# shellrow/nex

Measured on AMD Instinct MI355X. Metric: Mpkt/s + GiB/s device-resident parse+cksum, 64B & IMIX, 1/2/4/8 MI355X, higher is better.
Workload: dtype u8

## Files before the change

### nex_amd/csrc/frame_core.hpp

```cpp
#pragma once

#include <hip/hip_runtime.h>
#include <stdint.h>

#include "../../include/nexg.h"

#define NEXG_HD __host__ __device__ __forceinline__

namespace nexg {

NEXG_HD uint32_t ip_next_protocol_value(uint32_t n) {
    return (n <= 142u || n == 253u || n == 254u) ? n : 255u;
}

NEXG_HD uint32_t fold_complement(uint64_t t) {
    t = (t & 0xFFFFFFFFull) + (t >> 32);
    t = (t & 0xFFFFFFFFull) + (t >> 32);
    uint32_t s = (uint32_t)t;
    s = (s & 0xFFFFu) + (s >> 16);
    s = (s & 0xFFFFu) + (s >> 16);
    return (~s) & 0xFFFFu;
}

#define NEXG_NO_DEFER                                             \
// ... 68 lines not shown

#if defined(__HIP_DEVICE_COMPILE__)
#define NEXG_GLOBAL(T, p) reinterpret_cast<const __attribute__((address_space(1))) T*>(reinterpret_cast<uintptr_t>(p))
#else
#define NEXG_GLOBAL(T, p) reinterpret_cast<const T*>(p)
#endif

template <bool NT = false>
NEXG_HD uint4 load16(const void* p) {
    u32x4 v = NT ? __builtin_nontemporal_load(NEXG_GLOBAL(u32x4, p)) : *NEXG_GLOBAL(u32x4, p);
    return make_uint4(v.x, v.y, v.z, v.w);
}

template <bool NT = false>
NEXG_HD uint4 load16g(uint64_t addr) {
    return load16<NT>(reinterpret_cast<const void*>(addr));
}

NEXG_HD uint64_t global_le_sum(uint64_t A, uint64_t B) {
    uint64_t acc = 0;
    for (uint64_t d = A & ~15ull; d < B; d += 16) {
        const uint4 v = load16(reinterpret_cast<const void*>(d));
        uint32_t s = 0;
        if (d >= A && d + 16 <= B) {
            s = halves(v.x) + halves(v.y) + halves(v.z) + halves(v.w);
        } else {
            if (d + 0 < B) s += halves(v.x & range_mask(d + 0, A, B));
            if (d + 4 < B) s += halves(v.y & range_mask(d + 4, A, B));
            if (d + 8 < B) s += halves(v.z & range_mask(d + 8, A, B));
            if (d + 12 < B) s += halves(v.w & range_mask(d + 12, A, B));
        }
        acc += s;
    }
    return acc;
}

struct WinFrame {
    NEXG_NO_DEFER
    const uint8_t* slot;
    const uint8_t* g;
    uint32_t o;
    uint32_t wlen;

    NEXG_HD uint32_t u8(uint32_t i) const {
        return i < wlen ? (uint32_t)slot[o + i] : (uint32_t)g[i];
    }
    NEXG_HD uint64_t le_sum(uint32_t a, uint32_t b) const {
        uint64_t acc = 0;
        const uint32_t lb = b < wlen ? b : wlen;
        if (a < lb) {
            const uint32_t A = o + a, B = o + lb;
            const uint32_t* w = reinterpret_cast<const uint32_t*>(slot);
            uint32_t s = 0;
            for (uint32_t j = A & ~3u; j < B; j += 4) s += halves(w[j >> 2] & range_mask(j, A, B));
            acc = s;
        }
        const uint32_t ga = a > wlen ? a : wlen;
        if (ga < b) {
            const uint64_t base = reinterpret_cast<uint64_t>(g);
            acc += global_le_sum(base + ga, base + b);
        }
        return acc;
    }
};

struct SpanDeferred {
    uint32_t rng = 0;
    uint32_t t = 0;
    uint32_t meta = 0;
    NEXG_HD uint32_t which() const { return (meta >> 16) & 3u; }
    NEXG_HD uint32_t off() const { return rng & 0xFFFFu; }
    NEXG_HD uint32_t bytes() const { return rng >> 16; }
};

NEXG_HD uint32_t span_tail_end(uint32_t b12, uint32_t b16, uint32_t len, uint32_t opt_flags) {
    if (opt_flags & (NEXG_PARSE_FROM_IP | NEXG_PARSE_VLAN)) return len;
    const uint32_t et = ((b12 & 0xFFu) << 8) | ((b12 >> 8) & 0xFFu);
    const uint32_t e = et == 0x0800u ? 14u + (((b16 & 0xFFu) << 8) | ((b16 >> 8) & 0xFFu))
                     : et == 0x86DDu ? 54u + ((((b16 >> 16) & 0xFFu) << 8) | (b16 >> 24)) : 0u;
    return (e >= 84u && e < len) ? e : len;
}

#ifndef NEXG_SPAN_PROBE
#define NEXG_SPAN_PROBE(k, c)
#endif
#ifndef NEXG_SPAN_SLOT
#define NEXG_SPAN_SLOT 80
#endif
struct SpanFrame {
    static constexpr uint32_t kSlot = NEXG_SPAN_SLOT;
    static_assert(kSlot >= 80 && kSlot % 16 == 0, "the slot holds the 80-B fast-path window");
    static constexpr uint32_t kDefer = 64;
    const uint8_t* slot;
    const uint8_t* g;
    uint32_t tail_end;
    uint32_t parity;
    uint32_t tail;
    mutable SpanDeferred d{};
    mutable bool pend = false;

    NEXG_HD uint32_t u8(uint32_t i) const {
        NEXG_SPAN_PROBE(0, i >= kSlot);
        const uint8_t* p = i < kSlot ? slot + i : g + i;
        return *p;
    }
    NEXG_HD uint64_t le_sum(uint32_t a, uint32_t b) const {
        uint64_t acc = 0;
        const bool to_end = b == tail_end && tail_end > 80u && a <= 80u;
        const uint32_t lb = to_end ? 80u : b < kSlot ? b : kSlot;
        if (a < lb) {
            const uint32_t* w = reinterpret_cast<const uint32_t*>(slot);
            uint32_t s = 0;
            for (uint32_t j = a & ~3u; j < lb; j += 4) s += halves(w[j >> 2] & range_mask(j, a, lb));
            acc = parity ? (uint64_t)s * 256u : (uint64_t)s;
        }
        const uint32_t ga = a > kSlot ? a : kSlot;
        if (!to_end && ga < b) {
            const uint64_t base = reinterpret_cast<uint64_t>(g);
            if (b - ga > kDefer && d.rng == 0) {
                d.rng = ga | (b - ga) << 16;
                pend = true;
            } else {
                NEXG_SPAN_PROBE(1, true);
                acc += global_le_sum(base + ga, base + b);
            }
        }
        if (to_end) acc += tail;
        return acc;
    }
    NEXG_HD void note_mult(uint32_t m) const {
        if (pend) d.meta = (m == 256u ? 1u : 0u) << 18 | 1u << 20;
        pend = false;
    }
    NEXG_HD void note_finish(uint64_t t, uint32_t stored, uint32_t which) const {
        if ((d.meta >> 20) && !d.which()) {
            t = (t & 0xFFFFFFFFull) + (t >> 32);
            d.t = (uint32_t)((t & 0xFFFFFFFFull) + (t >> 32));
            d.meta = (d.meta & (1u << 18)) | which << 16 | (stored & 0xFFFFu);
        }
    }
};

NEXG_HD void span_patch(const SpanDeferred& d, uint64_t range_sum, nexg_record& r) {
    const uint32_t calc = fold_complement((uint64_t)d.t + (((d.meta >> 18) & 1u) ? range_sum * 256u : range_sum));
    const uint32_t stored = d.meta & 0xFFFFu;
    if (d.which() == kCsumIp) {
        r.ip_csum_calc = (uint16_t)calc;
        r.flags = (r.flags & ~NEXG_C_IP_OK) | (calc == stored ? NEXG_C_IP_OK : 0u);
    } else {
        r.l4_csum_calc = (uint16_t)calc;
        r.flags = (r.flags & ~NEXG_C_L4_OK) | (calc == stored ? NEXG_C_L4_OK : 0u);
    }
}


template <class O>
NEXG_HD void parse_udp(const O& o, uint32_t base, uint32_t n,
                                          uint64_t pseudo, nexg_record& r) {
    r.flags |= NEXG_L_TRANSPORT;
    uint32_t ulen = n >= 8 ? o.be16(base + 4) : 0u;
    if (n < 8 || ulen < 8u || n < ulen) {
        set_payload(r, base, n);
        return;
    }
    uint32_t sp = o.be16(base), dp = o.be16(base + 2), cs = o.be16(base + 6);
    r.flags |= NEXG_L_UDP;
    r.l4_off = (uint16_t)base;
    r.src_port = (uint16_t)sp;
    r.dst_port = (uint16_t)dp;
    r.l4_length = (uint16_t)ulen;
    r.l4_csum = (uint16_t)cs;
    uint64_t t = pseudo + 17u + ulen + sp + dp + ulen + o.wsum(base + 8, base + ulen);
    o.finish(t, cs, kCsumL4, r);
    set_payload(r, base + 8, ulen - 8);
}

template <class O>
NEXG_HD void parse_tcp(const O& o, uint32_t base, uint32_t n,
                                          uint64_t pseudo, nexg_record& r) {
    r.flags |= NEXG_L_TRANSPORT;
    bool ok = n >= 20;
    uint32_t off_res = ok ? o.f.u8(base + 12) : 0u;
    uint32_t hl = (off_res >> 4) * 4u;
    ok = ok && hl >= 20u && n >= hl;
    uint32_t stop = hl, nopt = 0;
    if (ok) {
        uint32_t off = 20;
        while (off < hl) {
            uint32_t kind = o.f.u8(base + off);
            off += 1;
            if (kind == 0u) {
                nopt++;
                stop = off;
                break;
            }
            if (kind == 1u) {
                nopt++;
                continue;
            }
            if (off >= hl) { ok = false; break; }
            uint32_t l = o.f.u8(base + off);
            off += 1;
            if (l < 2u) { ok = false; break; }
            if (off + (l - 2u) > hl) { ok = false; break; }
            nopt++;
            off += l - 2u;
        }
    }
    if (!ok) {
        set_payload(r, base, n);
        return;
    }
    uint32_t sp = o.be16(base), dp = o.be16(base + 2);
    uint32_t seq_hi = o.be16(base + 4), seq_lo = o.be16(base + 6);
    uint32_t ack_hi = o.be16(base + 8), ack_lo = o.be16(base + 10);
    uint32_t flags = o.f.u8(base + 13);
    uint32_t win = o.be16(base + 14), cs = o.be16(base + 16), urg = o.be16(base + 18);
    r.flags |= NEXG_L_TCP;
    r.l4_off = (uint16_t)base;
    r.src_port = (uint16_t)sp;
    r.dst_port = (uint16_t)dp;
    r.tcp_seq = (seq_hi << 16) | seq_lo;
    r.tcp_ack = (ack_hi << 16) | ack_lo;
    r.l4_length = (uint16_t)hl;
    r.l4_type = (uint8_t)flags;
    r.l4_code = (uint8_t)off_res;
    r.tcp_window = (uint16_t)win;
    r.tcp_urg = (uint16_t)urg;
    r.l4_nopt = (uint8_t)nopt;
    r.l4_csum = (uint16_t)cs;
    uint32_t hl_ser = 20u + ((stop - 20u + 3u) & ~3u);
    uint32_t len_ser = hl_ser + (n - hl);
    uint64_t t = pseudo + 6u + len_ser + sp + dp + seq_hi + seq_lo + ack_hi + ack_lo +
                 ((((hl_ser >> 2) << 4) | (off_res & 0xFu)) << 8 | flags) + win + urg +
                 o.wsum(base + 20, base + stop) + o.wsum(base + hl, base + n);
    o.finish(t, cs, kCsumL4, r);
    set_payload(r, base + hl, n - hl);
}

template <class O>
NEXG_HD void parse_icmp(const O& o, uint32_t base, uint32_t n,
                                           bool v6, uint64_t pseudo, nexg_record& r) {
    if (n < 8) {
        set_payload(r, base, n);
        return;
    }
    uint32_t tc = o.be16(base), cs = o.be16(base + 2);
    r.flags |= v6 ? NEXG_L_ICMPV6 : NEXG_L_ICMP;
    r.l4_off = (uint16_t)base;
    r.l4_type = (uint8_t)(tc >> 8);
    r.l4_code = (uint8_t)tc;
    r.l4_csum = (uint16_t)cs;
    uint64_t t = (v6 ? pseudo + 58u + n : 0ull) + tc + o.wsum(base + 4, base + n);
    o.finish(t, cs, kCsumL4, r);
    set_payload(r, base + 4, n - 4);
}


template <class O>
NEXG_HD uint32_t parse_ipv4(const O& o, uint32_t l3, uint32_t len,
                                               bool strict, nexg_record& r) {
    const uint32_t n = len - l3;
    r.flags |= NEXG_L_IP;
    uint32_t err = 0, ctx = 0, ea = 0, eb = 0, hl = 0, total = 0;
    uint32_t b0 = n >= 20u ? o.f.u8(l3) : 0u;
    if (n < 20u) { err = NEXG_ERR_BUFFER_TOO_SHORT; ctx = NEXG_CTX_IPV4_PACKET; ea = 20u; eb = n; }
    else if ((b0 >> 4) != 4u) { err = NEXG_ERR_MALFORMED; ctx = NEXG_CTX_IPV4_VERSION; }
    else if ((b0 & 15u) < 5u) { err = NEXG_ERR_INVALID_LENGTH; ctx = NEXG_CTX_IPV4_HEADER_LENGTH; ea = b0 & 15u; }
    else {
        hl = (b0 & 15u) * 4u;
        if (hl > n) { err = NEXG_ERR_TRUNCATED; ctx = NEXG_CTX_IPV4_HEADER; ea = hl; eb = n; }
        else {
            uint32_t declared = o.be16(l3 + 2);
            uint32_t eff = declared ? declared : n;
            if (eff < hl) { err = NEXG_ERR_INVALID_LENGTH; ctx = NEXG_CTX_IPV4_TOTAL_LENGTH; ea = declared; }
            else if (strict && eff > n) { err = NEXG_ERR_TRUNCATED; ctx = NEXG_CTX_IPV4_PACKET; ea = eff; eb = n; }
            else total = eff < n ? eff : n;
        }
    }
    uint32_t stop = hl, nopt = 0;
    if (!err) {
        uint32_t i = 20;
        while (i < hl) {
            uint32_t num = o.f.u8(l3 + i) & 0x1Fu;
            if (num == 0u) { nopt++; stop = i + 1; break; }
            if (num == 1u) { nopt++; i++; continue; }
            if (i + 2u > hl) {
                if (strict) { err = NEXG_ERR_MALFORMED; ctx = NEXG_CTX_IPV4_OPTIONS; }
                stop = i;
                break;
            }
            uint32_t l = o.f.u8(l3 + i + 1);
            if (l < 2u || i + l > hl) {
                if (strict) { err = NEXG_ERR_INVALID_LENGTH; ctx = NEXG_CTX_IPV4_OPTION_LENGTH; ea = l; }
                stop = i;
                break;
            }
            nopt++;
            i += l;
        }
    }
    if (err) {
        if (!strict) return 0u;
        r.l4_type = (uint8_t)ctx;
        r.ip_src = ea;
        r.ip_dst = eb;
// ... 609 lines not shown
```

### nex_amd/csrc/parse_kernels.hpp

```cpp
#pragma once

#include "frame_core.hpp"
#include "nexg_internal.hpp"

namespace nexg {

constexpr uint32_t kTile = 256;

#ifndef NEXG_DESC_MODE
#define NEXG_DESC_MODE 2
#endif
constexpr uint32_t kApron = NEXG_SPAN_SLOT > 96 ? NEXG_SPAN_SLOT : 96;

struct GlobalFrame {
    NEXG_NO_DEFER
    const uint8_t* g;
    NEXG_HD uint32_t u8(uint32_t i) const { return g[i]; }
    NEXG_HD uint64_t le_sum(uint32_t a, uint32_t b) const {
        const uint64_t base = reinterpret_cast<uint64_t>(g);
        return global_le_sum(base + a, base + b);
    }
};

__device__ __forceinline__ uint32_t wave_incl_scan(uint32_t v) {
// ... 365 lines not shown
    }
    if (!__all(fits)) {
        if (have) *handoff_slot<OUT>(a, idx) = (uint32_t)global_le_sum(myA, myA + len - kLaneWin);
        return;
    }
    acc[lane] = 0;
    const uint32_t incl = wave_incl_scan(np);
    pfx[lane] = incl - np;
    const uint32_t total = __shfl(incl, 63, 64);
    if (lane == 63) pfx[64] = total;
    wave_lds_sync();
    const uint32_t grp = lane >> 4, gl = lane & 15u;
    const uint32_t pb = (uint32_t)((uint64_t)total * grp / 4u);
    const uint32_t pe = (uint32_t)((uint64_t)total * (grp + 1u) / 4u);
    const uint8_t* wb = reinterpret_cast<const uint8_t*>(wbase);
    if (pb < pe) {
        uint32_t lo = 0, hi = 64;
        while (hi - lo > 1) {
            const uint32_t mid = (lo + hi) >> 1;
            if (pfx[mid] <= pb) lo = mid; else hi = mid;
        }
        uint32_t fi = lo;
        uint32_t cf = lo, ce = pfx[lo + 1];
        uint32_t ca = tail_a[lo], cb = tail_b[lo];
        uint32_t cpb = (ca & ~(kPiece - 1)) - pfx[lo] * kPiece;
        uint32_t run = 0;
        for (uint32_t p0 = pb; p0 < pe; p0 += PU) {
            uint4 v[PU];
            uint32_t C[PU], AA[PU], BB[PU], F[PU];
#pragma unroll
            for (uint32_t u = 0; u < PU; u++) {
                const uint32_t pp = p0 + u;
                while (pp < pe && pp >= ce) {
                    cf++;
                    ce = pfx[cf + 1];
                    ca = tail_a[cf];
                    cb = tail_b[cf];
                    cpb = (ca & ~(kPiece - 1)) - pfx[cf] * kPiece;
                }
                F[u] = cf;
                AA[u] = ca;
                BB[u] = cb;
                C[u] = cpb + pp * kPiece + 16u * gl;
            }
#pragma unroll
            for (uint32_t u = 0; u < PU; u++) {
                v[u] = make_uint4(0, 0, 0, 0);
                if (p0 + u < pe && C[u] < BB[u] && C[u] + 16u > AA[u]) v[u] = load16<true>(wb + C[u]);
            }
#pragma unroll
            for (uint32_t u = 0; u < PU; u++) {
                if (p0 + u >= pe) break;
                if (F[u] != fi) {
                    uint32_t s = run;
                    s += __shfl_xor(s, 8, 16);
                    s += __shfl_xor(s, 4, 16);
                    s += __shfl_xor(s, 2, 16);
                    s += __shfl_xor(s, 1, 16);
                    if (gl == 0 && s) atomicAdd(&acc[fi], s);
                    run = 0;
                    fi = F[u];
                }
                const uint32_t c = C[u], A = AA[u], B = BB[u];
                if (c < B && c + 16u > A) {
                    if (c >= A && c + 16u <= B) {
                        run += halves(v[u].x) + halves(v[u].y) + halves(v[u].z) + halves(v[u].w);
                    } else {
                        if (c + 0 < B) run += halves(v[u].x & range_mask(c + 0, A, B));
                        if (c + 4 < B) run += halves(v[u].y & range_mask(c + 4, A, B));
                        if (c + 8 < B) run += halves(v[u].z & range_mask(c + 8, A, B));
                        if (c + 12 < B) run += halves(v[u].w & range_mask(c + 12, A, B));
                    }
                }
            }
        }
        uint32_t s = run;
        s += __shfl_xor(s, 8, 16);
        s += __shfl_xor(s, 4, 16);
        s += __shfl_xor(s, 2, 16);
        s += __shfl_xor(s, 1, 16);
        if (gl == 0 && s) atomicAdd(&acc[fi], s);
    }
    wave_lds_sync();
    if (have) *handoff_slot<OUT>(a, idx) = acc[lane];
}

template <int OUT>
__global__ __launch_bounds__(256) void k_parse_lane80(ParseArgs a) {
    const uint64_t idx = (uint64_t)blockIdx.x * kTile + threadIdx.x;
    const bool valid = idx < a.count;
    if (!sparse_like(OUT) && !valid) return;
    uint64_t off = 0;
    uint32_t len = 0;
    nexg_record r{};
    const bool ext = valid && frame_extent(a, idx, off, len);
    if (valid && !ext) r.flags = (uint32_t)NEXG_ERR_BAD_EXTENT << NEXG_STATUS_SHIFT;
    const uint64_t abs = reinterpret_cast<uint64_t>(a.data) + off;
    const uint64_t dend = reinterpret_cast<uint64_t>(a.data) + a.data_bytes;
    bool done = !ext;
    if (ext && abs + kLaneWin <= dend) {
        const uint32_t tail = len > kLaneWin ? *handoff_slot<OUT>(a, idx) : 0u;
        const uint64_t a16 = abs & ~15ull;
        const uint32_t q = (uint32_t)(abs >> 2) & 3u, sh = (uint32_t)abs & 3u;
        uint32_t u[24];
#pragma unroll
        for (int k = 0; k < 6; k++) {
            const uint4 v = (k < 5 || a16 + 80u < dend) ? load16<true>(reinterpret_cast<const void*>(a16 + 16u * k))
                                                        : make_uint4(0, 0, 0, 0);
            u[4 * k] = v.x; u[4 * k + 1] = v.y; u[4 * k + 2] = v.z; u[4 * k + 3] = v.w;
        }
        uint32_t d[21];
#pragma unroll
        for (int j = 0; j < 21; j++) d[j] = q == 0 ? u[j] : q == 1 ? u[j + 1] : q == 2 ? u[j + 2] : u[j + 3];
        uint32_t w[20];
#pragma unroll
        for (int k = 0; k < 20; k++) w[k] = __builtin_amdgcn_alignbyte(d[k + 1], d[k], sh);
        done = fast_canonical80(w, len, a.opt_flags, (uint64_t)tail << (8u * (sh & 1u)), len, r);
    }
    if (!done) {
        GlobalFrame f{a.data + off};
        parse_frame(f, (uint32_t)(abs & 1u), len, a.opt_flags, a.ip_offset, r);
    }
    store_out<OUT>(a, idx, valid, r);
}

}

namespace nexg {


NEXG_HD uint32_t chunk_le_sum(const uint4& v) {
    return halves_acc(v.w, halves_acc(v.z, halves_acc(v.y, halves_acc(v.x, 0u))));
}

NEXG_HD uint32_t chunk_prefix_sum(const uint8_t* c, uint32_t m) {
    const uint4 v = *reinterpret_cast<const uint4*>(c);
    auto msk = [&](uint32_t d) {
        return m >= 4u * d + 4u ? 0xFFFFFFFFu : (m <= 4u * d ? 0u : ((1u << (8u * (m - 4u * d))) - 1u));
    };
    return halves_acc(v.w & msk(3), halves_acc(v.z & msk(2), halves_acc(v.y & msk(1), halves(v.x & msk(0)))));
}

NEXG_HD uint32_t chunk_range_sum(const uint4& v, uint64_t c, uint64_t A, uint64_t B) {
    if (c >= B || c + 16u <= A) return 0u;
    if (c >= A && c + 16u <= B) return chunk_le_sum(v);
    uint32_t s = halves(v.x & range_mask(c, A, B));
    if (c + 4 < B) s += halves(v.y & range_mask(c + 4, A, B));
    if (c + 8 < B) s += halves(v.z & range_mask(c + 8, A, B));
    if (c + 12 < B) s += halves(v.w & range_mask(c + 12, A, B));
    return s;
}

constexpr uint32_t kBuckets = 9;
NEXG_HD uint32_t span_bucket(uint32_t w3, uint32_t w5, uint32_t opt_flags) {
    if (opt_flags & NEXG_PARSE_FROM_IP) return 8u;
    const uint32_t et = ((w3 & 0xFFu) << 8) | ((w3 >> 8) & 0xFFu);
    if (et == 0x0800u) {
        const uint32_t p = w5 >> 24;
        return p == 6u ? 0u : p == 17u ? 1u : p == 1u ? 2u : 3u;
    }
    if (et == 0x86DDu) {
        const uint32_t p = w5 & 0xFFu;
        return p == 6u ? 4u : p == 17u ? 5u : p == 58u ? 6u : 7u;
    }
    return 8u;
}

__device__ __forceinline__ uint32_t wave_incl_scan_dpp(uint32_t v) {
    v += (uint32_t)__builtin_amdgcn_update_dpp(0, (int)v, 0x111, 0xF, 0xF, false);
    v += (uint32_t)__builtin_amdgcn_update_dpp(0, (int)v, 0x112, 0xF, 0xF, false);
    v += (uint32_t)__builtin_amdgcn_update_dpp(0, (int)v, 0x114, 0xF, 0xF, false);
    v += (uint32_t)__builtin_amdgcn_update_dpp(0, (int)v, 0x118, 0xF, 0xF, false);
    v += (uint32_t)__builtin_amdgcn_update_dpp(0, (int)v, 0x142, 0xA, 0xF, false);
    v += (uint32_t)__builtin_amdgcn_update_dpp(0, (int)v, 0x143, 0xC, 0xF, false);
    return v;
}

#define NEXG_SPAN_STAMP(k) \
    do { if constexpr (TIMING) { if (t == 0) a.stamps[blockIdx.x * 8ull + (k)] = __builtin_amdgcn_s_memtime(); } } while (0)
#define NEXG_SPAN_RTSTAMP(k) \
    do { if constexpr (TIMING) { if (t == 0) a.stamps[blockIdx.x * 8ull + (k)] = __builtin_amdgcn_s_memrealtime(); } } while (0)

#ifndef NEXG_SPAN_NT
#define NEXG_SPAN_NT true
#endif
#ifndef NEXG_SPAN_PF
#define NEXG_SPAN_PF 0
#endif
#ifndef NEXG_SPAN_DEPTH
#define NEXG_SPAN_DEPTH 1
#endif
template <int OUT, int NB = 1, uint32_t SUB = 16384, int WPE = 1, bool TIMING = false>
__global__ __launch_bounds__(256) __attribute__((amdgpu_waves_per_eu(WPE))) void k_parse_span(ParseArgs a) {
    constexpr uint32_t kStage = kApron + SUB + kApron > kTile * SpanFrame::kSlot ? kApron + SUB + kApron
                                                                                 : kTile * SpanFrame::kSlot;
    __shared__ __attribute__((aligned(16))) uint8_t s_bytes[NB][kStage];
    __shared__ __attribute__((aligned(16))) uint32_t s_pfx[NB][(SUB / 16u) + 4];
    __shared__ uint32_t s_wsum[NB][4];
    __shared__ uint64_t s_span[2];
    __shared__ uint32_t s_hist[2 * kBuckets + 1];
    const uint32_t t = threadIdx.x, lane = t & 63u, wv = t >> 6;
    NEXG_SPAN_RTSTAMP(6);
    NEXG_SPAN_STAMP(0);
    const uint64_t f0 = tile_index(a.tile_order) * kTile;
    const uint64_t idx = f0 + t;
    const uint32_t nf = a.count - f0 < kTile ? (uint32_t)(a.count - f0) : kTile;
    const uint64_t base = reinterpret_cast<uint64_t>(a.data);
    uint64_t off = 0;
    uint32_t len = 0;
    const bool have = t < nf;
    if (OUT == NEXG_OUT_SPARSE && a.grouped_heads && lane == 0 && have) a.grouped_heads[idx >> 6] = NEXG_GROUPED_TILE_RUN;
    if (OUT == NEXG_OUT_GROUPED && lane == 0 && have) reinterpret_cast<uint8_t*>(a.out)[idx >> 6] = 0;
#if NEXG_SPAN_PF
    uint64_t pfv = 0;
    const uint64_t pfb = (uint64_t)blockIdx.x + 8ull * NEXG_SPAN_PF;
    if (a.offsets && !a.lengths && !(a.hints & NEXG_FRAMES_OFFSETS32) && pfb < gridDim.x && t < 33u) {
        const uint64_t pg = tile_of((uint32_t)pfb, gridDim.x, a.tile_order) * kTile + 8u * t;
        if (pg <= a.count) pfv = NEXG_GLOBAL(uint64_t, a.offsets)[pg];
    }
#endif
    const bool ok = have && frame_extent(a, idx, off, len);
    if (t == 0) s_span[0] = off;
    if (t == nf - 1) s_span[1] = off + len;
    __syncthreads();
    const uint64_t lo = s_span[0], hi = s_span[1];
    const uint64_t A0 = (base + lo) & ~15ull;
    const uint32_t span = (uint32_t)(((base + hi + 15u) & ~15ull) - A0);
    constexpr int CPT = SUB / 4096u;
    uint4 cur[CPT];
#if NEXG_SPAN_DEPTH == 2
    uint4 nxt[CPT];
#endif
    auto fetch = [&](uint32_t S, uint4 (&v)[CPT]) {
#pragma unroll
        for (int i = 0; i < CPT; i++) {
            const uint32_t c = S + 16u * (t + 256u * i);
            v[i] = c < span ? load16g<NEXG_SPAN_NT>(A0 + c) : make_uint4(0, 0, 0, 0);
        }
    };
    const bool plausible = hi >= lo && hi <= a.data_bytes && hi - lo <= (1ull << 30);
    if (plausible) {
        fetch(0, cur);
#if NEXG_SPAN_DEPTH == 2
        fetch(SUB, nxt);
#endif
    }
    const bool inside = !have || (ok && off >= lo && off + len <= hi);
    const bool span_ok = __syncthreads_and(inside) && plausible;
    NEXG_SPAN_STAMP(1);
    nexg_record r{};
    if (!span_ok) {
        if (have) {
            if (!ok) {
                r.flags = (uint32_t)NEXG_ERR_BAD_EXTENT << NEXG_STATUS_SHIFT;
            } else {
                GlobalFrame f{a.data + off};
                parse_frame(f, (uint32_t)((base + off) & 1u), len, a.opt_flags, a.ip_offset, r);
            }
        }
        store_out<OUT>(a, idx, have, r);
        NEXG_SPAN_STAMP(5);
        NEXG_SPAN_RTSTAMP(7);
        return;
    }
    const uint32_t hr = (uint32_t)(base + off - A0);
    const bool want_tail = have && len > kLaneWin;
    const uint32_t sh = (uint32_t)((base + off) & 3u);
    uint32_t qa = 0, qb = 0, run = 0;
    uint32_t qend = len;
    constexpr uint32_t NW = SpanFrame::kSlot / 4u + 1u;
    uint32_t u[NW];
#pragma unroll
    for (int j = 0; j < (int)NW; j++) u[j] = 0;

    uint32_t buf = 0;
    auto sub_tile = [&](const uint32_t S, uint4 (&v)[CPT]) {
        uint8_t* sb = s_bytes[buf] + kApron;
        uint32_t* sp = s_pfx[buf];
        if (S > 0 && t >= kTile - kApron / 16u) {
            const uint8_t* prev = s_bytes[NB == 2 ? buf ^ 1u : buf] + kApron + SUB - kApron;
            *reinterpret_cast<uint4*>(sb - kApron + 16u * (t - (kTile - kApron / 16u))) =
                *reinterpret_cast<const uint4*>(prev + 16u * (t - (kTile - kApron / 16u)));
        }
#pragma unroll
        for (int i = 0; i < CPT; i++) {
            const uint32_t c = t + 256u * i;
            *reinterpret_cast<uint4*>(sb + 16u * c) = v[i];
            sp[c] = chunk_le_sum(v[i]);
        }
        const uint32_t E = S + SUB;
        if (S + NEXG_SPAN_DEPTH * SUB < span) fetch(S + NEXG_SPAN_DEPTH * SUB, v);
        __syncthreads();
        uint32_t cs[CPT];
        uint32_t own = 0;
#pragma unroll
        for (int i = 0; i < CPT; i++) own += (cs[i] = sp[CPT * t + i]);
        const uint32_t incl = wave_incl_scan_dpp(own);
        if (lane == 63u) s_wsum[buf][wv] = incl;
        __syncthreads();
        const uint4 ws = *reinterpret_cast<const uint4*>(s_wsum[buf]);
        const uint32_t wbase = (wv > 0 ? ws.x : 0u) + (wv > 1 ? ws.y : 0u) + (wv > 2 ? ws.z : 0u);
        const uint32_t total = ws.x + ws.y + ws.z + ws.w;
        uint32_t ex = wbase + incl - own;
#pragma unroll
        for (int i = 0; i < CPT; i++) {
            sp[CPT * t + i] = ex;
            ex += cs[i];
        }
        if (t == 0) sp[(SUB / 16u)] = total;
        __syncthreads();
        const bool last = E >= span;
        auto q_at = [&](uint32_t d) {
            const uint32_t c = d >> 4, m = d & 15u;
            return run + sp[c] + (m ? chunk_prefix_sum(sb + 16u * c, m) : 0u);
        };
        const int dh = (int)((hr & ~3u) - S);
        constexpr int kWin = (int)SpanFrame::kSlot;
        if (have && dh >= -kWin && (dh <= (int)SUB - kWin - 4 || (last && dh < (int)SUB))) {
#pragma unroll
            for (int j = 0; j < (int)NW; j++) u[j] = *reinterpret_cast<const uint32_t*>(sb + dh + 4 * j);
            qend = span_tail_end(__builtin_amdgcn_alignbyte(u[4], u[3], sh),
                                 __builtin_amdgcn_alignbyte(u[5], u[4], sh), len, a.opt_flags);
        }
        const uint32_t da = hr + kLaneWin - S, db = hr + qend - S;
        if (want_tail && (da < SUB || (last && da == SUB))) qa = q_at(da);
        if (have && (db < SUB || (last && db == SUB))) qb = q_at(db);
        run += total;
        if (NB == 1) __syncthreads();
    };
#if NEXG_SPAN_DEPTH == 2
    static_assert(NB == 1, "depth 2 runs on one stage buffer");
    for (uint32_t S = 0; S < span; S += 2u * SUB) {
        sub_tile(S, cur);
        if (S + SUB < span) sub_tile(S + SUB, nxt);
    }
#else
    for (uint32_t S = 0; S < span; S += SUB, buf = NB == 2 ? buf ^ 1u : 0u) sub_tile(S, cur);
#endif
    if (NB == 2) __syncthreads();
#if NEXG_SPAN_PF
    if (pfv == ~0ull) s_hist[0] = 1u;
#endif
    NEXG_SPAN_STAMP(2);
    uint8_t* const slots = &s_bytes[0][0];
    uint32_t code = 0, key = 0;
    bool gen = false;
    const uint32_t tq = want_tail ? qb - qa : 0u;
    if (have) {
        uint32_t w[20];
#pragma unroll
        for (int k = 0; k < 20; k++) w[k] = __builtin_amdgcn_alignbyte(u[k + 1], u[k], sh);
        const uint64_t tail = (sh & 1u) ? (uint64_t)tq * 256u : (uint64_t)tq;
        if (fast_canonical80(w, len, a.opt_flags, tail, qend, r)) {
            if (sparse_like(OUT)) code = canonical80_code(r);
            if (OUT == NEXG_OUT_RECORD) stage_record(slots + SpanFrame::kSlot * t, r);
        } else {
            gen = true;
            constexpr int NS = (int)SpanFrame::kSlot / 4;
            uint32_t x[NS];
#pragma unroll
            for (int k = 0; k < NS; k++) {
                const uint32_t v = k < 20 ? w[k] : __builtin_amdgcn_alignbyte(u[k + 1], u[k], sh);
                x[k] = 4u * k < len ? (v & range_mask(4u * k, 0, len)) : 0u;
            }
            key = span_bucket(x[3], x[5], a.opt_flags);
#pragma unroll
            for (int k = 0; k < NS / 4; k++)
                reinterpret_cast<uint4*>(slots + SpanFrame::kSlot * t)[k] =
                    make_uint4(x[4 * k], x[4 * k + 1], x[4 * k + 2], x[4 * k + 3]);
        }
    }
    NEXG_SPAN_STAMP(3);
    if (__syncthreads_or(gen)) {
        if (t < kBuckets) s_hist[t] = 0;
        __syncthreads();
        const uint32_t rank = gen ? atomicAdd(&s_hist[key], 1u) : 0u;
        __syncthreads();
        if (t == 0) {
            uint32_t acc = 0;
            for (uint32_t k = 0; k < kBuckets; k++) {
                const uint32_t c = s_hist[k];
                s_hist[kBuckets + k] = acc;
                acc += c;
            }
            s_hist[2 * kBuckets] = acc;
        }
        __syncthreads();
        uint4* const items = reinterpret_cast<uint4*>(&s_pfx[0][0]);
        if (gen) items[s_hist[kBuckets + key] + rank] = make_uint4(hr, len | qend << 16, tq, t);
        const uint32_t ngen = s_hist[2 * kBuckets];
        __syncthreads();
        const bool work = t < ngen;
        nexg_record rr{};
        SpanDeferred dfr{};
        uint32_t owner = 0, ghr = 0;
        if (work) {
            const uint4 it = items[t];
            ghr = it.x;
            owner = it.w;
            SpanFrame f{slots + SpanFrame::kSlot * owner, reinterpret_cast<const uint8_t*>(A0 + ghr), it.y >> 16,
                        ghr & 1u, it.z};
            parse_frame(f, ghr & 1u, it.y & 0xFFFFu, a.opt_flags, a.ip_offset, rr);
            dfr = f.d;
        }
        uint32_t mine = 0;
        const uint32_t grp = lane >> 4, gl = lane & 15u;
        for (uint64_t m = __ballot(dfr.which() != 0u); m;) {
            const uint64_t cur = m;
            uint64_t rest = cur;
            uint32_t pick = 64u;
#pragma unroll
            for (uint32_t k = 0; k < 4; k++) {
                const uint32_t b = rest ? (uint32_t)__builtin_ctzll(rest) : 64u;
                pick = k == grp ? b : pick;
                rest &= rest - 1;
            }
            m = rest;
            const int src = (int)(pick & 63u);
            const uint32_t rg = (uint32_t)__shfl((int)dfr.rng, src, 64);
            const uint64_t A = A0 + (uint32_t)__shfl((int)ghr, src, 64) + (rg & 0xFFFFu);
            const uint64_t B = pick < 64u ? A + (rg >> 16) : A;
            uint32_t s = 0;
            for (uint64_t c = (A & ~15ull) + 16u * gl; c < B; c += 1024u) {
                uint4 v[4];
#pragma unroll
                for (uint32_t k = 0; k < 4; k++)
                    v[k] = c + 256u * k < B ? load16(reinterpret_cast<const void*>(c + 256u * k)) : make_uint4(0, 0, 0, 0);
#pragma unroll
                for (uint32_t k = 0; k < 4; k++) s += chunk_range_sum(v[k], c + 256u * k, A, B);
            }
            s += __shfl_xor(s, 8, 16);
            s += __shfl_xor(s, 4, 16);
            s += __shfl_xor(s, 2, 16);
            s += __shfl_xor(s, 1, 16);
            const uint32_t rk = (uint32_t)__builtin_popcountll(cur & ((1ull << lane) - 1ull));
            const uint32_t tot = (uint32_t)__shfl((int)s, (int)((rk & 3u) << 4), 64);
            if (((cur >> lane) & 1ull) && rk < 4u) mine = tot;
        }
        if (dfr.which()) span_patch(dfr, mine, rr);
        if (work) {
            uint8_t* os = slots + SpanFrame::kSlot * owner;
            if (OUT == NEXG_OUT_RECORD) {
                stage_record(os, rr);
            } else {
                const uint32_t c = sparse_like(OUT) ? sparse_encode(rr, a.opt_flags, a.ip_offset) : 0u;
                *reinterpret_cast<uint4*>(os) =
                    make_uint4(rr.flags, (uint32_t)rr.payload_off | ((uint32_t)rr.payload_len << 16), c, 0u);
            }
        }
        __syncthreads();
        if (gen && OUT != NEXG_OUT_RECORD) {
            const uint4 v = *reinterpret_cast<const uint4*>(slots + SpanFrame::kSlot * t);
            r.flags = v.x;
            r.payload_off = (uint16_t)v.y;
            r.payload_len = (uint16_t)(v.y >> 16);
            code = v.z;
        }
    }
    NEXG_SPAN_STAMP(4);
    if (sparse_like(OUT)) store_sparse_coded<OUT, false>(a, idx, have, r, code);
    else if (OUT == NEXG_OUT_DESC && NEXG_DESC_MODE == 2) {
        if (have) stage_desc(slots + SpanFrame::kSlot * t, r);
        __syncthreads();
        copy_out_descs<SpanFrame::kSlot>(slots, a.out, f0, nf);
    } else if (OUT != NEXG_OUT_RECORD) store_out<OUT>(a, idx, have, r);
    if (OUT == NEXG_OUT_RECORD) {
        static_assert(kStage >= kTile * SpanFrame::kSlot, "record staging needs kTile slots");
        __syncthreads();
        copy_out_records<SpanFrame::kSlot>(slots, a.out, f0, nf);
    }
    NEXG_SPAN_STAMP(5);
    NEXG_SPAN_RTSTAMP(7);
}



}
```

Before: 115,200.

## Parse rare generic-path frames with a whole wave per frame when few

```diff
diff --git a/nex_amd/csrc/frame_core.hpp b/nex_amd/csrc/frame_core.hpp
--- a/nex_amd/csrc/frame_core.hpp
+++ b/nex_amd/csrc/frame_core.hpp
@@ -244,6 +244,116 @@
         r.flags = (r.flags & ~NEXG_C_L4_OK) | (calc == stored ? NEXG_C_L4_OK : 0u);
     }
 }
+
+constexpr uint32_t kWaveImage = 256;
+constexpr uint32_t kWaveSlot = 80;
+
+NEXG_HD void wave_image_load(uint32_t j, uint64_t fa, uint32_t lim, uint64_t span_end, uint32_t& g0, uint32_t& g1,
+                             uint32_t& mask) {
+    g0 = g1 = mask = 0u;
+    if (4u * j < kWaveSlot || 4u * j >= lim) return;
+    const uint64_t p = (fa + 4u * j) & ~3ull;
+    mask = range_mask(4u * j, 0, lim);
+    g0 = *NEXG_GLOBAL(uint32_t, p);
+    if ((fa & 3u) && p + 4u < span_end) g1 = *NEXG_GLOBAL(uint32_t, p + 4u);
+}
+NEXG_HD uint32_t wave_image_join(uint32_t g0, uint32_t g1, uint32_t mask, uint32_t sh) {
+#if defined(__HIP_DEVICE_COMPILE__)
+    return __builtin_amdgcn_alignbyte(g1, g0, sh) & mask;
+#else
+    return (sh ? (g0 >> (8u * sh)) | (g1 << (32u - 8u * sh)) : g0) & mask;
+#endif
+}
+NEXG_HD uint32_t wave_image_dword(uint32_t j, uint32_t slot_dword, uint64_t fa, uint32_t lim, uint64_t span_end) {
+    if (4u * j < kWaveSlot) return slot_dword;
+    uint32_t g0, g1, mask;
+    wave_image_load(j, fa, lim, span_end, g0, g1, mask);
+    return wave_image_join(g0, g1, mask, (uint32_t)(fa & 3u));
+}
+
+NEXG_HD uint32_t wave_lane_range_sum(uint32_t lane, uint64_t A, uint64_t B) {
+    uint32_t s = 0;
+    for (uint64_t c = (A & ~15ull) + 16u * lane; c < B; c += 1024u) {
+        const uint4 v = load16(reinterpret_cast<const void*>(c));
+        if (c >= A && c + 16u <= B) {
+            s = halves_acc(v.w, halves_acc(v.z, halves_acc(v.y, halves_acc(v.x, s))));
+        } else {
+            if (c + 4 > A) s += halves(v.x & range_mask(c, A, B));
+            if (c + 4 < B && c + 8 > A) s += halves(v.y & range_mask(c + 4, A, B));
+            if (c + 8 < B && c + 12 > A) s += halves(v.z & range_mask(c + 8, A, B));
+            if (c + 12 < B) s += halves(v.w & range_mask(c + 12, A, B));
+        }
+    }
+    return s;
+}
+
+struct WaveFrame {
+    NEXG_NO_DEFER
+    uint32_t img;
+    uint32_t g0, g1, gmask;
+    uint32_t lane;
+    const uint32_t* lanes;
+    const uint8_t* g;
+    uint32_t tail_end;
+    uint32_t parity;
+    uint32_t tail;
+
+#if defined(__HIP_DEVICE_COMPILE__)
+    __device__ __forceinline__ uint32_t high() const {
+        return wave_image_join(g0, g1, gmask, (uint32_t)(reinterpret_cast<uint64_t>(g) & 3u));
+    }
+    __device__ __forceinline__ uint32_t dword(uint32_t j) const {
+        if (j < kWaveSlot / 4u) return (uint32_t)__builtin_amdgcn_readlane((int)img, (int)j);
+        return (uint32_t)__builtin_amdgcn_readlane((int)high(), (int)j);
+    }
+    __device__ __forceinline__ static uint32_t wave_sum(uint32_t v) {
+        v += (uint32_t)__builtin_amdgcn_update_dpp(0, (int)v, 0x111, 0xF, 0xF, false);
+        v += (uint32_t)__builtin_amdgcn_update_dpp(0, (int)v, 0x112, 0xF, 0xF, false);
+        v += (uint32_t)__builtin_amdgcn_update_dpp(0, (int)v, 0x114, 0xF, 0xF, false);
+        v += (uint32_t)__builtin_amdgcn_update_dpp(0, (int)v, 0x118, 0xF, 0xF, false);
+        v += (uint32_t)__builtin_amdgcn_update_dpp(0, (int)v, 0x142, 0xA, 0xF, false);
+        v += (uint32_t)__builtin_amdgcn_update_dpp(0, (int)v, 0x143, 0xC, 0xF, false);
+        return (uint32_t)__builtin_amdgcn_readlane((int)v, 63);
+    }
+#else
+    uint32_t dword(uint32_t j) const { return lanes[j]; }
+#endif
+    NEXG_HD static uint32_t image_part(uint32_t j, uint32_t w, uint32_t a, uint32_t lb) {
+        return (4u * j < lb && 4u * j + 4u > a) ? halves(w & range_mask(4u * j, a, lb)) : 0u;
+    }
+
+    NEXG_HD uint32_t u8(uint32_t i) const {
+        if (i < kWaveImage) return (dword(i >> 2) >> (8u * (i & 3u))) & 0xFFu;
+        return (uint32_t)*NEXG_GLOBAL(uint8_t, g + i);
+    }
+    NEXG_HD uint64_t le_sum(uint32_t a, uint32_t b) const {
+        uint64_t acc = 0;
+        const bool to_end = b == tail_end && tail_end > 80u && a <= 80u;
+        const uint32_t lb = to_end ? 80u : b < kWaveImage ? b : kWaveImage;
+        if (a < lb) {
+#if defined(__HIP_DEVICE_COMPILE__)
+            const uint32_t s = lb <= kWaveSlot ? wave_sum(image_part(lane, img, a, lb))
+                                               : wave_sum(image_part(lane, lane < kWaveSlot / 4u ? img : high(), a, lb));
+#else
+            uint32_t s = 0;
+            for (uint32_t j = 0; j < 64u; j++) s += image_part(j, lanes[j], a, lb);
+#endif
+            acc = parity ? (uint64_t)s * 256u : (uint64_t)s;
+        }
+        const uint32_t ga = a > kWaveImage ? a : kWaveImage;
+        if (to_end) {
+            acc += tail;
+        } else if (ga < b) {
+            const uint64_t base = reinterpret_cast<uint64_t>(g);
+#if defined(__HIP_DEVICE_COMPILE__)
+            acc += wave_sum(wave_lane_range_sum(lane, base + ga, base + b));
+#else
+            for (uint32_t j = 0; j < 64u; j++) acc += wave_lane_range_sum(j, base + ga, base + b);
+#endif
+        }
+        return acc;
+    }
+};
 
 
 template <class O>
diff --git a/nex_amd/csrc/parse_kernels.hpp b/nex_amd/csrc/parse_kernels.hpp
--- a/nex_amd/csrc/parse_kernels.hpp
+++ b/nex_amd/csrc/parse_kernels.hpp
@@ -541,6 +541,10 @@
 }
 
 constexpr uint32_t kBuckets = 9;
+#ifndef NEXG_SPAN_WAVE_GEN
+#define NEXG_SPAN_WAVE_GEN 4
+#endif
+constexpr uint32_t kWaveGen = NEXG_SPAN_WAVE_GEN;
 NEXG_HD uint32_t span_bucket(uint32_t w3, uint32_t w5, uint32_t opt_flags) {
     if (opt_flags & NEXG_PARSE_FROM_IP) return 8u;
     const uint32_t et = ((w3 & 0xFFu) << 8) | ((w3 >> 8) & 0xFFu);
@@ -588,6 +592,7 @@
     __shared__ uint32_t s_wsum[NB][4];
     __shared__ uint64_t s_span[2];
     __shared__ uint32_t s_hist[2 * kBuckets + 1];
+    __shared__ uint64_t s_gmask[kTile / 64u];
     const uint32_t t = threadIdx.x, lane = t & 63u, wv = t >> 6;
     NEXG_SPAN_RTSTAMP(6);
     NEXG_SPAN_STAMP(0);
@@ -760,81 +765,136 @@
         }
     }
     NEXG_SPAN_STAMP(3);
-    if (__syncthreads_or(gen)) {
-        if (t < kBuckets) s_hist[t] = 0;
-        __syncthreads();
-        const uint32_t rank = gen ? atomicAdd(&s_hist[key], 1u) : 0u;
-        __syncthreads();
-        if (t == 0) {
-            uint32_t acc = 0;
-            for (uint32_t k = 0; k < kBuckets; k++) {
-                const uint32_t c = s_hist[k];
-                s_hist[kBuckets + k] = acc;
-                acc += c;
-            }
-            s_hist[2 * kBuckets] = acc;
-        }
-        __syncthreads();
-        uint4* const items = reinterpret_cast<uint4*>(&s_pfx[0][0]);
-        if (gen) items[s_hist[kBuckets + key] + rank] = make_uint4(hr, len | qend << 16, tq, t);
-        const uint32_t ngen = s_hist[2 * kBuckets];
-        __syncthreads();
-        const bool work = t < ngen;
-        nexg_record rr{};
-        SpanDeferred dfr{};
-        uint32_t owner = 0, ghr = 0;
-        if (work) {
-            const uint4 it = items[t];
-            ghr = it.x;
-            owner = it.w;
-            SpanFrame f{slots + SpanFrame::kSlot * owner, reinterpret_cast<const uint8_t*>(A0 + ghr), it.y >> 16,
-                        ghr & 1u, it.z};
-            parse_frame(f, ghr & 1u, it.y & 0xFFFFu, a.opt_flags, a.ip_offset, rr);
-            dfr = f.d;
-        }
-        uint32_t mine = 0;
-        const uint32_t grp = lane >> 4, gl = lane & 15u;
-        for (uint64_t m = __ballot(dfr.which() != 0u); m;) {
-            const uint64_t cur = m;
-            uint64_t rest = cur;
-            uint32_t pick = 64u;
-#pragma unroll
-            for (uint32_t k = 0; k < 4; k++) {
-                const uint32_t b = rest ? (uint32_t)__builtin_ctzll(rest) : 64u;
-                pick = k == grp ? b : pick;
-                rest &= rest - 1;
-            }
-            m = rest;
-            const int src = (int)(pick & 63u);
-            const uint32_t rg = (uint32_t)__shfl((int)dfr.rng, src, 64);
-            const uint64_t A = A0 + (uint32_t)__shfl((int)ghr, src, 64) + (rg & 0xFFFFu);
-            const uint64_t B = pick < 64u ? A + (rg >> 16) : A;
-            uint32_t s = 0;
-            for (uint64_t c = (A & ~15ull) + 16u * gl; c < B; c += 1024u) {
-                uint4 v[4];
-#pragma unroll
-                for (uint32_t k = 0; k < 4; k++)
-                    v[k] = c + 256u * k < B ? load16(reinterpret_cast<const void*>(c + 256u * k)) : make_uint4(0, 0, 0, 0);
-#pragma unroll
-                for (uint32_t k = 0; k < 4; k++) s += chunk_range_sum(v[k], c + 256u * k, A, B);
-            }
-            s += __shfl_xor(s, 8, 16);
-            s += __shfl_xor(s, 4, 16);
-            s += __shfl_xor(s, 2, 16);
-            s += __shfl_xor(s, 1, 16);
-            const uint32_t rk = (uint32_t)__builtin_popcountll(cur & ((1ull << lane) - 1ull));
-            const uint32_t tot = (uint32_t)__shfl((int)s, (int)((rk & 3u) << 4), 64);
-            if (((cur >> lane) & 1ull) && rk < 4u) mine = tot;
-        }
-        if (dfr.which()) span_patch(dfr, mine, rr);
-        if (work) {
-            uint8_t* os = slots + SpanFrame::kSlot * owner;
-            if (OUT == NEXG_OUT_RECORD) {
-                stage_record(os, rr);
-            } else {
-                const uint32_t c = sparse_like(OUT) ? sparse_encode(rr, a.opt_flags, a.ip_offset) : 0u;
-                *reinterpret_cast<uint4*>(os) =
-                    make_uint4(rr.flags, (uint32_t)rr.payload_off | ((uint32_t)rr.payload_len << 16), c, 0u);
+    uint4* const items = reinterpret_cast<uint4*>(&s_pfx[0][0]);
+    {
+        const uint64_t bm = __ballot(gen);
+        if (lane == 0) s_gmask[wv] = bm;
+        if (gen) items[t] = make_uint4(hr, len | qend << 16, tq, t);
+    }
+    __syncthreads();
+    uint64_t gmask[kTile / 64u];
+    uint32_t ngu = 0;
+#pragma unroll
+    for (uint32_t w = 0; w < kTile / 64u; w++) {
+        const uint64_t m = s_gmask[w];
+        gmask[w] = (uint64_t)(uint32_t)__builtin_amdgcn_readfirstlane((int)(uint32_t)m) |
+                   (uint64_t)(uint32_t)__builtin_amdgcn_readfirstlane((int)(uint32_t)(m >> 32)) << 32;
+        ngu += (uint32_t)__builtin_popcountll(gmask[w]);
+    }
+    if (ngu) {
+        if (ngu <= kWaveGen) {
+            for (uint32_t i = (uint32_t)__builtin_amdgcn_readfirstlane((int)wv); i < ngu; i += kTile / 64u) {
+                uint32_t k = i, wow = 0;
+#pragma unroll
+                for (uint32_t w = 0; w < kTile / 64u; w++) {
+                    uint64_t m = gmask[w];
+                    const uint32_t c = (uint32_t)__builtin_popcountll(m);
+                    if (k < c) {
+                        for (; k; k--) m &= m - 1;
+                        wow = 64u * w + (uint32_t)__builtin_ctzll(m);
+                        k = ~0u;
+                    } else if (k != ~0u) {
+                        k -= c;
+                    }
+                }
+                const uint4 it = items[wow];
+                const uint32_t whr = (uint32_t)__builtin_amdgcn_readfirstlane((int)it.x);
+                const uint32_t wle = (uint32_t)__builtin_amdgcn_readfirstlane((int)it.y);
+                const uint32_t wtq = (uint32_t)__builtin_amdgcn_readfirstlane((int)it.z);
+                const uint32_t wlen = wle & 0xFFFFu;
+                uint8_t* os = slots + SpanFrame::kSlot * wow;
+                uint32_t g0, g1, gm;
+                wave_image_load(lane, A0 + whr, wlen < kWaveImage ? wlen : kWaveImage, A0 + span, g0, g1, gm);
+                const uint32_t sd = lane < kWaveSlot / 4u ? reinterpret_cast<const uint32_t*>(os)[lane] : 0u;
+                WaveFrame f{sd, g0, g1, gm, lane, nullptr, reinterpret_cast<const uint8_t*>(A0 + whr), wle >> 16,
+                            whr & 1u, wtq};
+                nexg_record wr{};
+                parse_frame(f, whr & 1u, wlen, a.opt_flags, a.ip_offset, wr);
+                if (lane == 0) {
+                    if (OUT == NEXG_OUT_RECORD) {
+                        stage_record(os, wr);
+                    } else {
+                        const uint32_t c = sparse_like(OUT) ? sparse_encode(wr, a.opt_flags, a.ip_offset) : 0u;
+                        *reinterpret_cast<uint4*>(os) =
+                            make_uint4(wr.flags, (uint32_t)wr.payload_off | ((uint32_t)wr.payload_len << 16), c, 0u);
+                    }
+                }
+            }
+        } else {
+            if (t < kBuckets) s_hist[t] = 0;
+            __syncthreads();
+            const uint32_t rank = gen ? atomicAdd(&s_hist[key], 1u) : 0u;
+            __syncthreads();
+            if (t == 0) {
+                uint32_t acc = 0;
+                for (uint32_t k = 0; k < kBuckets; k++) {
+                    const uint32_t c = s_hist[k];
+                    s_hist[kBuckets + k] = acc;
+                    acc += c;
+                }
+                s_hist[2 * kBuckets] = acc;
+            }
+            __syncthreads();
+            if (gen) items[s_hist[kBuckets + key] + rank] = make_uint4(hr, len | qend << 16, tq, t);
+            const uint32_t ngen = s_hist[2 * kBuckets];
+            __syncthreads();
+            const bool work = t < ngen;
+            nexg_record rr{};
+            SpanDeferred dfr{};
+            uint32_t owner = 0, ghr = 0;
+            if (work) {
+                const uint4 it = items[t];
+                ghr = it.x;
+                owner = it.w;
+                SpanFrame f{slots + SpanFrame::kSlot * owner, reinterpret_cast<const uint8_t*>(A0 + ghr), it.y >> 16,
+                            ghr & 1u, it.z};
+                parse_frame(f, ghr & 1u, it.y & 0xFFFFu, a.opt_flags, a.ip_offset, rr);
+                dfr = f.d;
+            }
+            uint32_t mine = 0;
+            const uint32_t grp = lane >> 4, gl = lane & 15u;
+            for (uint64_t m = __ballot(dfr.which() != 0u); m;) {
+                const uint64_t cur = m;
+                uint64_t rest = cur;
+                uint32_t pick = 64u;
+#pragma unroll
+                for (uint32_t k = 0; k < 4; k++) {
+                    const uint32_t b = rest ? (uint32_t)__builtin_ctzll(rest) : 64u;
+                    pick = k == grp ? b : pick;
+                    rest &= rest - 1;
+                }
+                m = rest;
+                const int src = (int)(pick & 63u);
+                const uint32_t rg = (uint32_t)__shfl((int)dfr.rng, src, 64);
+                const uint64_t A = A0 + (uint32_t)__shfl((int)ghr, src, 64) + (rg & 0xFFFFu);
+                const uint64_t B = pick < 64u ? A + (rg >> 16) : A;
+                uint32_t s = 0;
+                for (uint64_t c = (A & ~15ull) + 16u * gl; c < B; c += 1024u) {
+                    uint4 v[4];
+#pragma unroll
+                    for (uint32_t k = 0; k < 4; k++)
+                        v[k] = c + 256u * k < B ? load16(reinterpret_cast<const void*>(c + 256u * k)) : make_uint4(0, 0, 0, 0);
+#pragma unroll
+                    for (uint32_t k = 0; k < 4; k++) s += chunk_range_sum(v[k], c + 256u * k, A, B);
+                }
+                s += __shfl_xor(s, 8, 16);
+                s += __shfl_xor(s, 4, 16);
+                s += __shfl_xor(s, 2, 16);
+                s += __shfl_xor(s, 1, 16);
+                const uint32_t rk = (uint32_t)__builtin_popcountll(cur & ((1ull << lane) - 1ull));
+                const uint32_t tot = (uint32_t)__shfl((int)s, (int)((rk & 3u) << 4), 64);
+                if (((cur >> lane) & 1ull) && rk < 4u) mine = tot;
+            }
+            if (dfr.which()) span_patch(dfr, mine, rr);
+            if (work) {
+                uint8_t* os = slots + SpanFrame::kSlot * owner;
+                if (OUT == NEXG_OUT_RECORD) {
+                    stage_record(os, rr);
+                } else {
+                    const uint32_t c = sparse_like(OUT) ? sparse_encode(rr, a.opt_flags, a.ip_offset) : 0u;
+                    *reinterpret_cast<uint4*>(os) =
+                        make_uint4(rr.flags, (uint32_t)rr.payload_off | ((uint32_t)rr.payload_len << 16), c, 0u);
+                }
             }
         }
         __syncthreads();
```

New measurement: 115,200 (median of 3 runs). No clear change (+0.0%).
